# gtonkinhill/tracs

Hardware: NVIDIA B200
Metric: site-pair comparisons/s (P*L/t) (higher is better)
Workload: dtype u32 bit-planes (int32 counts), f64 likelihood

## Files before the change

### tracs_b200/csrc/sweep.cu

```cuda
#include <cub/cub.cuh>

#include <algorithm>
#include <memory>
#include <stdexcept>
#include <type_traits>

#include "common.cuh"
#include "trans.cuh"

namespace tracs {

static inline uint64_t round_up(uint64_t x, uint64_t m) { return (x + m - 1) / m * m; }

constexpr int PACK_THREADS = 256;
constexpr int PACK_SCHUNK = 256;
constexpr int PACK_BATCH = 4;

__device__ __forceinline__ uint32_t bsel(uint32_t a, uint32_t b, uint32_t m) { return (a & m) | (b & ~m); }

__device__ __forceinline__ uint32_t nibbles_all_ones(uint32_t x) {
  uint32_t t = x & (x >> 1);
  t &= (t >> 2);
  t &= 0x11111111u;
  t = (t | (t >> 3)) & 0x03030303u;
// ... 386 lines not shown
__global__ void k_site_sources(const uint32_t *__restrict__ vlist, uint32_t V, const uint32_t *__restrict__ elist, uint32_t VE,
                               uint32_t *__restrict__ src, uint32_t *__restrict__ late) {
  const uint32_t v = blockIdx.x * blockDim.x + threadIdx.x;
  if (v >= V) return;
  const uint32_t site = vlist[v];
  uint32_t a = 0, b = VE;
  while (a < b) {
    const uint32_t mid = (a + b) >> 1;
    if (elist[mid] < site) a = mid + 1; else b = mid;
  }
  if (a < VE && elist[a] == site) {
    src[v] = a;
  } else {
    src[v] = 0x80000000u | (v - a);
    late[v - a] = site;
  }
}

__device__ __forceinline__ uint32_t slice_bits4(uint32_t r, int b) {
  return (((r >> b) & 0x01010101u) * 0x01020408u) >> 24;
}
__device__ __forceinline__ uint4 slice_word(const uint4 &q0, const uint4 &q1) {
  const uint32_t r[8] = {q0.x, q0.y, q0.z, q0.w, q1.x, q1.y, q1.z, q1.w};
  uint32_t o[4];
#pragma unroll
  for (int b = 0; b < 4; ++b) {
    uint32_t v = 0;
#pragma unroll
    for (int k = 0; k < 8; ++k) v |= (slice_bits4(r[k], b) & 0xFu) << (4 * k);
    o[b] = v;
  }
  return make_uint4(o[0], o[1], o[2], o[3]);
}
__device__ __forceinline__ bool slice_ambiguous(const uint4 &p) {
  const uint32_t two = (p.x & p.y) | (p.x & p.z) | (p.x & p.w) | (p.y & p.z) | (p.y & p.w) | (p.z & p.w);
  return (two & ~(p.x & p.y & p.z & p.w)) != 0u;
}

__global__ void __launch_bounds__(256)
k_slice(const uint8_t *__restrict__ X, uint64_t XP, const uint8_t *__restrict__ X2, uint64_t X2P, const uint32_t *__restrict__ src,
        uint64_t V, uint64_t n, uint4 *__restrict__ planes, uint64_t Npad, uint4 *__restrict__ planesT, uint64_t Wp, uint32_t schunk,
        uint32_t *__restrict__ amb_flag) {
  const uint32_t lane = threadIdx.x & 31;
  const uint64_t w0 = ((uint64_t)blockIdx.x * 8 + (threadIdx.x >> 5)) * 2;
  if (w0 * 32 >= V) return;
  const uint64_t s0 = (uint64_t)blockIdx.y * schunk, s1 = min(n, s0 + schunk);
  bool fast = (w0 + 2) * 32 <= V;
  uint32_t base = 0;
  if (fast) {
    const uint32_t a = src[w0 * 32 + lane], b = src[w0 * 32 + 32 + lane];
    base = __shfl_sync(0xFFFFFFFFu, a, 0);
    fast = __all_sync(0xFFFFFFFFu, a == base + lane && b == base + 32 + lane) && !(base & 0x80000000u) && (base & 15u) == 0;
  }
  if (fast) {
    bool amb = false, hasn = false;
    for (uint64_t s = s0 + lane; s < s1; s += 32) {
      const uint4 *row = reinterpret_cast<const uint4 *>(X + s * XP + base);
      const uint4 q0 = __ldg(row), q1 = __ldg(row + 1), q2 = __ldg(row + 2), q3 = __ldg(row + 3);
      const uint4 pa = slice_word(q0, q1), pb = slice_word(q2, q3);
      amb |= slice_ambiguous(pa) | slice_ambiguous(pb);
      hasn |= ((pa.x & pa.y & pa.z & pa.w) | (pb.x & pb.y & pb.z & pb.w)) != 0u;
      planes[w0 * Npad + s] = pa;
      planes[(w0 + 1) * Npad + s] = pb;
      planesT[s * Wp + w0] = pa;
      planesT[s * Wp + w0 + 1] = pb;
    }
    if (__any_sync(0xFFFFFFFFu, amb) && lane == 0) atomicOr(amb_flag, 1u);
    if (__any_sync(0xFFFFFFFFu, hasn) && lane == 0) atomicOr(amb_flag, 2u);
    return;
  }
  for (uint64_t w = w0; w < w0 + 2 && w * 32 < V; ++w) {
    const uint64_t v = w * 32 + lane;
    const bool live = v < V;
    const uint32_t sv = live ? src[v] : 0u;
    const uint8_t *col = (sv & 0x80000000u) ? X2 + (sv & 0x7FFFFFFFu) : X + sv;
    const uint64_t cp = (sv & 0x80000000u) ? X2P : XP;
    constexpr int GB = 8;
    for (uint64_t sb = s0; sb < s1; sb += GB) {
      uint8_t mk[GB];
#pragma unroll
      for (int t = 0; t < GB; ++t) mk[t] = (live && sb + t < s1) ? __ldg(col + (sb + t) * cp) : (uint8_t)15;
#pragma unroll
      for (int t = 0; t < GB; ++t) {
        const uint64_t s = sb + t;
        if (s >= s1) break;
        const uint32_t m = mk[t];
        if (__any_sync(0xFFFFFFFFu, m != 15u && (m & (m - 1)) != 0u) && lane == 0) atomicOr(amb_flag, 1u);
        if (__any_sync(0xFFFFFFFFu, live && m == 15u) && lane == 0) atomicOr(amb_flag, 2u);
        const uint32_t A = __ballot_sync(0xFFFFFFFFu, m & 1);
        const uint32_t C = __ballot_sync(0xFFFFFFFFu, m & 2);
        const uint32_t G = __ballot_sync(0xFFFFFFFFu, m & 4);
        const uint32_t T = __ballot_sync(0xFFFFFFFFu, m & 8);
        if (lane == 0) {
          const uint4 o = make_uint4(A, C, G, T);
          planes[w * Npad + s] = o;
          planesT[s * Wp + w] = o;
        }
      }
    }
  }
}

struct SweepArgs {
  const uint4 *planes;
  uint32_t Wp;
  uint32_t Npad;
  uint32_t n, i_end, j_start;
  int32_t dist;
  const uint32_t *rb_list;
  const uint32_t *tile_prefix;
  uint32_t n_rb;
  uint32_t n_tiles;
  uint32_t cb_min;
  const uint2 *tile_table;
  const uint32_t *tc_ncnt;
  union {
    struct {
      unsigned long long *counter;
      uint64_t *keys;
      uint32_t *dvals;
      unsigned long long cap;
    };
    struct {
      int32_t *dense;
      uint64_t dense_ld;
      uint32_t dense_col0;
      uint32_t dense_mirror;
    };
  };
  uint32_t one;
};

__device__ __forceinline__ uint32_t smem_u32(const void *p) { return (uint32_t)__cvta_generic_to_shared(p); }
__device__ __forceinline__ void mbar_init(uint64_t *bar, uint32_t count) {
  asm volatile("mbarrier.init.shared::cta.b64 [%0], %1;" ::"r"(smem_u32(bar)), "r"(count) : "memory");
}
__device__ __forceinline__ void mbar_expect_tx(uint64_t *bar, uint32_t bytes) {
  asm volatile("mbarrier.arrive.expect_tx.shared::cta.b64 _, [%0], %1;" ::"r"(smem_u32(bar)), "r"(bytes) : "memory");
}
__device__ __forceinline__ void mbar_wait(uint64_t *bar, uint32_t parity) {
  uint32_t done;
  do {
    asm volatile(
        "{\n"
        ".reg .pred p;\n"
        "mbarrier.try_wait.parity.shared::cta.b64 p, [%1], %2;\n"
        "selp.u32 %0, 1, 0, p;\n"
        "}\n"
        : "=r"(done)
        : "r"(smem_u32(bar)), "r"(parity)
        : "memory");
  } while (!done);
}
__device__ __forceinline__ void bulk_g2s(void *dst, const void *src, uint32_t bytes, uint64_t *bar) {
  asm volatile("cp.async.bulk.shared::cluster.global.mbarrier::complete_tx::bytes [%0], [%1], %2, [%3];" ::"r"(
                   smem_u32(dst)),
               "l"(src), "r"(bytes), "r"(smem_u32(bar))
               : "memory");
}

__global__ void k_tile_table(const uint32_t *__restrict__ rb_list, const uint32_t *__restrict__ tile_prefix, uint32_t n_rb, uint32_t cb_min,
                             uint32_t n_tiles, uint2 *__restrict__ table) {
  const uint32_t tile = blockIdx.x * blockDim.x + threadIdx.x;
  if (tile >= n_tiles) return;
  uint32_t lo = 0, hi = n_rb;
  while (hi - lo > 1) {
    const uint32_t mid = (lo + hi) >> 1;
    if (tile_prefix[mid] <= tile) lo = mid; else hi = mid;
  }
  const uint32_t rb = rb_list[lo];
  table[tile] = make_uint2(rb, max(rb, cb_min) + (tile - tile_prefix[lo]));
}

constexpr int SWEEP_THREADS = 256;
constexpr int STAGE_U4 = KC * TILE;
constexpr uint32_t PREFILTER_WORDS = 64;
static inline uint32_t prefilter_words(int64_t dist) {
  const uint64_t w = ((uint64_t)(dist + 1) * 8 + 31) / 32;
  return (uint32_t)std::min<uint64_t>(PREFILTER_WORDS, std::max<uint64_t>(16, round_up(w, 16)));
}
static inline uint32_t first_window(int64_t dist) {
  if (dist < 22) return 4;
  if (dist < 43) return 8;
  return prefilter_words(dist);
}
constexpr uint32_t TC_MIN_WORDS = 17;
static inline uint32_t next_window(uint32_t pw) { return pw < 8 ? 8 : pw < 16 ? 16 : (pw < PREFILTER_WORDS ? PREFILTER_WORDS : 0); }
constexpr size_t SWEEP_SMEM = (size_t)STAGES * 2 * STAGE_U4 * sizeof(uint4);

extern __shared__ __align__(128) uint8_t smem_raw[];

template <bool DENSE>
__global__ void __launch_bounds__(SWEEP_THREADS, 1) k_sweep(const SweepArgs a) {
  extern __shared__ __align__(128) uint8_t smem_raw[];
  uint4 *srow = reinterpret_cast<uint4 *>(smem_raw);
  uint4 *scol = srow + (size_t)STAGES * STAGE_U4;
  __shared__ __align__(8) uint64_t full[STAGES];
  __shared__ uint2 s_tile[4];
  constexpr uint32_t HB_CAP = 1024, HB_FLUSH = 512, HB_LANE_MAX = 4;
  __shared__ uint64_t hb_key[HB_CAP];
  __shared__ uint32_t hb_val[HB_CAP];
  __shared__ uint32_t hb_count;
  __shared__ unsigned long long hb_base;

  const uint32_t tid = threadIdx.x;
  const uint32_t tx = tid & 15, ty = tid >> 4;
  if (tid == 0) {
    for (int s = 0; s < STAGES; ++s) mbar_init(&full[s], 1);
    asm volatile("fence.mbarrier_init.release.cluster;" ::: "memory");
    hb_count = 0;
  }
  __syncthreads();
  auto flush_hits = [&]() {
    const uint32_t cnt = hb_count;
    if (tid == 0) hb_base = cnt ? atomicAdd(a.counter, (unsigned long long)cnt) : 0ull;
    __syncthreads();
    const unsigned long long base = hb_base;
    for (uint32_t e = tid; e < cnt; e += SWEEP_THREADS)
      if (base + e < a.cap) {
        a.keys[base + e] = hb_key[e];
        a.dvals[base + e] = hb_val[e];
      }
    __syncthreads();
    if (tid == 0) hb_count = 0;
    __syncthreads();
  };

  const uint32_t nk = (a.Wp + KC - 1) / KC;
  const int kc_used = a.Wp < (uint32_t)KC ? (int)a.Wp : KC;
  const uint32_t one = a.one;
  const uint32_t my_tiles = blockIdx.x < a.n_tiles ? (a.n_tiles - blockIdx.x + gridDim.x - 1) / gridDim.x : 0;
  const uint32_t total_chunks = my_tiles * nk;
  const uint32_t warp_id = tid >> 5, lane_id = tid & 31;
  uint32_t iss_g = 0, iss_t = 0, iss_c = 0, iss_slot = 0;
  uint2 rc_next = my_tiles ? __ldg(a.tile_table + blockIdx.x) : make_uint2(0u, 0u);
  auto issue = [&]() {
    const uint2 rc = rc_next;
    uint64_t *bar = &full[iss_slot];
    if (lane_id == 0) {
      if (iss_c == 0) s_tile[iss_t & 3] = rc;
      mbar_expect_tx(bar, 2u * STAGE_U4 * (uint32_t)sizeof(uint4));
    }
    __syncwarp();
    if (lane_id < 2u * KC) {
      const uint32_t kk = lane_id >> 1;
      const bool is_col = (lane_id & 1u) != 0u;
      const uint4 *src = a.planes + (size_t)(is_col ? rc.y : rc.x) * TILE + (size_t)(iss_c * KC + kk) * a.Npad;
      uint4 *dst = (is_col ? scol : srow) + (size_t)iss_slot * STAGE_U4 + kk * TILE;
      bulk_g2s(dst, src, TILE * sizeof(uint4), bar);
    }
    ++iss_g;
    iss_slot = iss_slot + 1 == (uint32_t)STAGES ? 0u : iss_slot + 1;
    if (++iss_c == nk) {
      iss_c = 0;
      if (++iss_t < my_tiles) rc_next = __ldg(a.tile_table + blockIdx.x + (size_t)iss_t * gridDim.x);
    }
  };
  if (warp_id == 0)
    while (iss_g < (uint32_t)STAGES && iss_g < total_chunks) issue();
  __syncthreads();
  uint32_t it = 0;
  uint32_t t_iter = 0;

  for (uint32_t tile = blockIdx.x; tile < a.n_tiles; tile += gridDim.x, ++t_iter) {
    const uint2 rc = s_tile[t_iter & 3];
    const uint32_t rb = rc.x, cb = rc.y;

    uint32_t acc[8][8];
#pragma unroll
    for (int i = 0; i < 8; ++i)
#pragma unroll
      for (int j = 0; j < 8; ++j) acc[i][j] = 0;

    for (uint32_t c = 0; c < nk; ++c, ++it) {
      const uint32_t slot = it % STAGES;
      mbar_wait(&full[slot], (it / STAGES) & 1u);
      const uint4 *pr = srow + (size_t)slot * STAGE_U4 + ty;
      const uint4 *pc = scol + (size_t)slot * STAGE_U4 + tx;
#pragma unroll 2
      for (int kk = 0; kk < kc_used; ++kk) {
        uint4 r[8];
#pragma unroll
        for (int i = 0; i < 8; ++i) r[i] = pr[kk * TILE + i * 16];
#pragma unroll
        for (int j = 0; j < 8; ++j) {
          const uint4 cv = pc[kk * TILE + j * 16];
#pragma unroll
          for (int i = 0; i < 8; ++i) {
            const uint32_t m = (r[i].x & cv.x) | (r[i].y & cv.y) | (r[i].z & cv.z) | (r[i].w & cv.w);
            acc[i][j] = __popc(m) * one + acc[i][j];
          }
        }
      }
      const int want_flush = c + 1 == nk && *(volatile uint32_t *)&hb_count > HB_FLUSH;
      const int do_flush = __syncthreads_or(want_flush);
      if (warp_id == 0 && iss_g < total_chunks) issue();
      if (do_flush) flush_hits();
    }

    const uint32_t total_bits = a.Wp * 32u;
    if constexpr (DENSE) {
#pragma unroll
      for (int i = 0; i < 8; ++i) {
        const uint32_t gi = rb * TILE + i * 16 + ty;
#pragma unroll
        for (int j = 0; j < 8; ++j) {
          const uint32_t gj = cb * TILE + j * 16 + tx;
          if (gi < a.i_end && gj < a.n && gj > gi && gj >= a.j_start) {
            const int32_t d = (int32_t)(total_bits - acc[i][j]);
            a.dense[(uint64_t)gi * a.dense_ld + (gj - a.dense_col0)] = d;
            if (a.dense_mirror) a.dense[(uint64_t)gj * a.dense_ld + gi] = d;
          }
        }
        if (a.dense_mirror && cb == rb && tx == ty && gi < a.n) a.dense[(uint64_t)gi * a.dense_ld + gi] = 0;
      }
      continue;
    }
    const uint32_t lane = tid & 31;
    uint32_t rmax[8];
#pragma unroll
    for (int i = 0; i < 8; ++i) {
      uint32_t m = acc[i][0];
#pragma unroll
      for (int j = 1; j < 8; ++j) m = max(m, acc[i][j]);
      rmax[i] = m;
    }
    uint32_t mx = rmax[0];
#pragma unroll
    for (int i = 1; i < 8; ++i) mx = max(mx, rmax[i]);
    const bool hit = (int32_t)(total_bits - mx) <= a.dist;
    const uint32_t hits = __ballot_sync(0xFFFFFFFFu, hit);
    if (!hits) continue;
    if (__popc(hits) <= 8) {
      if (hit) {
        uint32_t rowmask = 0;
#pragma unroll
        for (int i = 0; i < 8; ++i) rowmask |= ((int32_t)(total_bits - rmax[i]) <= a.dist ? 1u : 0u) << i;
        uint32_t parked = 0;
        while (rowmask) {
          const int i = __ffs(rowmask) - 1;
          rowmask &= rowmask - 1;
          uint32_t rv[8];
#pragma unroll
          for (int j = 0; j < 8; ++j) {
            uint32_t v = acc[0][j];
#pragma unroll
            for (int ii = 1; ii < 8; ++ii) v = i == ii ? acc[ii][j] : v;
            rv[j] = v;
          }
          const uint32_t gi = rb * TILE + (uint32_t)i * 16 + ty;
          uint32_t keepj = 0;
#pragma unroll
          for (int j = 0; j < 8; ++j) {
            const uint32_t gj = cb * TILE + j * 16 + tx;
            const bool ok = (int32_t)(total_bits - rv[j]) <= a.dist && gi < a.i_end && gj < a.n && gj > gi && gj >= a.j_start;
            keepj |= (ok ? 1u : 0u) << j;
          }
          while (keepj) {
            const int j = __ffs(keepj) - 1;
            keepj &= keepj - 1;
            uint32_t v = rv[0];
#pragma unroll
            for (int jj = 1; jj < 8; ++jj) v = j == jj ? rv[jj] : v;
            const uint64_t key = ((uint64_t)gi << 32) | (cb * TILE + (uint32_t)j * 16 + tx);
            if (parked < HB_LANE_MAX) {
              const uint32_t pos = atomicAdd(&hb_count, 1u);
              hb_key[pos] = key;
              hb_val[pos] = total_bits - v;
              ++parked;
            } else {
              const unsigned long long pos = atomicAdd(a.counter, 1ull);
              if (pos < a.cap) {
                a.keys[pos] = key;
                a.dvals[pos] = total_bits - v;
              }
            }
          }
        }
      }
      continue;
    }
    uint32_t cnt = 0;
    uint64_t keep = 0;
#pragma unroll
    for (int i = 0; i < 8; ++i) {
      const uint32_t gi = rb * TILE + i * 16 + ty;
#pragma unroll
      for (int j = 0; j < 8; ++j) {
        const uint32_t gj = cb * TILE + j * 16 + tx;
        const int32_t d = (int32_t)(total_bits - acc[i][j]);
        const bool ok = gi < a.i_end && gj < a.n && gj > gi && gj >= a.j_start && d <= a.dist;
        if (ok) {
          keep |= 1ull << (i * 8 + j);
          cnt++;
        }
      }
    }
    uint32_t incl = cnt;
#pragma unroll
    for (int o = 1; o < 32; o <<= 1) {
      uint32_t t = __shfl_up_sync(0xFFFFFFFFu, incl, o);
      if (lane >= (uint32_t)o) incl += t;
    }
    const uint32_t wtot = __shfl_sync(0xFFFFFFFFu, incl, 31);
    if (wtot) {
      unsigned long long base = 0;
      if (lane == 31) base = atomicAdd(a.counter, (unsigned long long)wtot);
      base = __shfl_sync(0xFFFFFFFFu, base, 31);
      unsigned long long pos = base + (incl - cnt);
#pragma unroll
      for (int i = 0; i < 8; ++i) {
#pragma unroll
        for (int j = 0; j < 8; ++j) {
          if ((keep >> (i * 8 + j)) & 1ull) {
            if (pos < a.cap) {
              const uint32_t gi = rb * TILE + i * 16 + ty;
              const uint32_t gj = cb * TILE + j * 16 + tx;
              a.keys[pos] = ((uint64_t)gi << 32) | gj;
              a.dvals[pos] = total_bits - acc[i][j];
            }
            pos++;
          }
        }
      }
    }
  }
  __syncthreads();
  flush_hits();
}

__global__ void k_expand(const uint64_t *__restrict__ keys, const uint32_t *__restrict__ dvals, uint64_t E,
                         uint64_t *__restrict__ rows, uint64_t *__restrict__ cols, uint64_t *__restrict__ dist) {
  uint64_t e = (uint64_t)blockIdx.x * blockDim.x + threadIdx.x;
  if (e >= E) return;
  uint64_t k = keys[e];
  rows[e] = k >> 32;
  cols[e] = k & 0xFFFFFFFFull;
  dist[e] = dvals[e];
}

__global__ void __launch_bounds__(256)
k_refine(const uint64_t *__restrict__ ckeys, const uint32_t *__restrict__ cdvals, uint64_t n_cand,
         const uint4 *__restrict__ planesT, uint32_t Wp, uint32_t w0, int32_t dist, unsigned long long *counter,
         uint64_t *__restrict__ keys, uint32_t *__restrict__ dvals) {
  const uint64_t e = ((uint64_t)blockIdx.x * blockDim.x + threadIdx.x) >> 5;
  const uint32_t lane = threadIdx.x & 31;
  if (e >= n_cand) return;
  const uint64_t k = ckeys[e];
  const uint4 *ri = planesT + (k >> 32) * Wp;
  const uint4 *rj = planesT + (k & 0xFFFFFFFFull) * Wp;
  uint32_t mism = 0;
#pragma unroll 4
  for (uint32_t w = w0 + lane; w < Wp; w += 32) {
    const uint4 x = __ldg(ri + w), y = __ldg(rj + w);
    mism += __popc(~((x.x & y.x) | (x.y & y.y) | (x.z & y.z) | (x.w & y.w)));
  }
#pragma unroll
  for (int o = 16; o > 0; o >>= 1) mism += __shfl_xor_sync(0xFFFFFFFFu, mism, o);
  if (lane == 0) {
    const uint32_t d = cdvals[e] + mism;
    if ((int32_t)d <= dist) {
      const unsigned long long pos = atomicAdd(counter, 1ull);
      keys[pos] = k;
      dvals[pos] = d;
    }
  }
}

__global__ void __launch_bounds__(256)
k_cand_trim(const uint64_t *__restrict__ keys, const uint32_t *__restrict__ dvals, uint64_t n_cand, const uint4 *__restrict__ planesT,
            uint32_t Wp, uint32_t w0, uint32_t extra, int32_t dist, uint8_t *__restrict__ flags) {
  const uint64_t e = (uint64_t)blockIdx.x * blockDim.x + threadIdx.x;
  if (e >= n_cand) return;
  const uint64_t k = keys[e];
  const uint4 *ri = planesT + (k >> 32) * Wp + w0, *rj = planesT + (k & 0xFFFFFFFFull) * Wp + w0;
  uint32_t d = dvals[e];
  for (uint32_t w = 0; w < extra && (int32_t)d <= dist; w += 4) {
#pragma unroll
    for (uint32_t q = 0; q < 4; ++q) {
      if (w + q < extra) {
        const uint4 x = __ldg(ri + w + q), y = __ldg(rj + w + q);
        d += __popc(~((x.x & y.x) | (x.y & y.y) | (x.z & y.z) | (x.w & y.w)));
      }
    }
  }
  flags[e] = (int32_t)d <= dist ? 1 : 0;
}

__global__ void __launch_bounds__(256)
k_snp_positions(const uint64_t *__restrict__ keys, uint64_t e0, uint64_t e1, const uint4 *__restrict__ planesT, uint32_t Wp,
                const uint32_t *__restrict__ site_idx, uint64_t V, const uint64_t *__restrict__ offs, uint64_t base,
                uint32_t *__restrict__ pos) {
  const uint64_t e = e0 + (((uint64_t)blockIdx.x * blockDim.x + threadIdx.x) >> 5);
  const uint32_t lane = threadIdx.x & 31;
  if (e >= e1) return;
  const uint64_t k = keys[e];
  const uint4 *ri = planesT + (k >> 32) * Wp;
  const uint4 *rj = planesT + (k & 0xFFFFFFFFull) * Wp;
  uint32_t *out = pos + (offs[e] - base);
  uint32_t written = 0;
  for (uint32_t w0 = 0; w0 < Wp; w0 += 32) {
    const uint32_t w = w0 + lane;
    uint32_t mis = 0;
    if (w < Wp) {
      const uint4 x = __ldg(ri + w), y = __ldg(rj + w);
      mis = ~((x.x & y.x) | (x.y & y.y) | (x.z & y.z) | (x.w & y.w));
    }
    const uint32_t c = __popc(mis);
    uint32_t incl = c;
#pragma unroll
    for (int o = 1; o < 32; o <<= 1) {
      const uint32_t t = __shfl_up_sync(0xFFFFFFFFu, incl, o);
      if (lane >= (uint32_t)o) incl += t;
    }
    uint32_t at = written + incl - c;
    while (mis) {
      const uint32_t b = __ffs(mis) - 1;
      mis &= mis - 1;
      const uint64_t v = (uint64_t)w * 32 + b;
      out[at++] = v < V ? site_idx[v] : 0u;
    }
    written += __shfl_sync(0xFFFFFFFFu, incl, 31);
  }
}

__global__ void __launch_bounds__(256)
k_filter_recomb(const uint32_t *__restrict__ dvals, uint64_t e0, uint64_t e1, const uint64_t *__restrict__ offs, uint64_t base,
                const uint32_t *__restrict__ pos, uint64_t L, const double *__restrict__ lg, uint32_t *__restrict__ filt) {
  const uint64_t e = e0 + (((uint64_t)blockIdx.x * blockDim.x + threadIdx.x) >> 5);
  const uint32_t lane = threadIdx.x & 31;
  if (e >= e1) return;
  const uint32_t d = dvals[e];
  if (d <= 1) {
    if (lane == 0) filt[e] = d;
    return;
  }
  const uint32_t *ps = pos + (offs[e] - base);
  const int aln = (int)L;
  const double dd = (double)d;
  const double p = dd / aln, thr = 0.05 / dd;
  int h = (int)(1.0 / p / 2.0 + 1);
  h = min(h, 5000);
  h = max(h, 50);
  const double lp = log(p), lq = log1p(-p);
  uint32_t kept = 0;
  for (uint32_t s = lane; s < d; s += 32) {
    const int i = (int)ps[s];
    const int left = max(0, i - h), right = min(aln, i + h + 1);
    uint32_t lo = 0, hi = s;
    while (lo < hi) { const uint32_t m = (lo + hi) >> 1; if ((int)ps[m] < left) lo = m + 1; else hi = m; }
    const uint32_t a = lo;
    lo = s; hi = d;
    while (lo < hi) { const uint32_t m = (lo + hi) >> 1; if ((int)ps[m] < right) lo = m + 1; else hi = m; }
    const uint32_t b = lo;
    const uint32_t cnt = b - a;
    if (cnt > 1) {
      const double n = (double)(int)(ps[b - 1] - ps[a] + 1), kk = (double)(int)cnt;
      double cdf;
      if (kk >= n) cdf = 1.0;
      else {
        cdf = 0.0;
        const int ni = (int)n;
        for (int t = 0; t <= (int)cnt; ++t)
          cdf += exp(lg[ni + 1] - lg[t + 1] - lg[ni - t + 1] + (double)t * lp + (double)(ni - t) * lq);
        if (cdf > 1.0) cdf = 1.0;
      }
      if (1.0 - cdf >= thr) kept++;
    } else {
      kept++;
    }
  }
#pragma unroll
  for (int o = 16; o > 0; o >>= 1) kept += __shfl_xor_sync(0xFFFFFFFFu, kept, o);
  if (lane == 0) filt[e] = kept;
}
__global__ void k_pack_edges(const uint64_t *__restrict__ keys, const uint32_t *__restrict__ dvals, const uint64_t *__restrict__ ncomp,
                             const double *__restrict__ p0, const double *__restrict__ eK, uint64_t E, uint8_t *__restrict__ out) {
  const uint64_t e = (uint64_t)blockIdx.x * blockDim.x + threadIdx.x;
  if (e >= E) return;
  uint32_t *u = reinterpret_cast<uint32_t *>(out);
  double *f = reinterpret_cast<double *>(out + 16 * E);
  const uint64_t k = keys[e];
  u[e] = (uint32_t)(k >> 32);
  u[E + e] = (uint32_t)k;
  u[2 * E + e] = dvals[e];
  u[3 * E + e] = ncomp ? (uint32_t)ncomp[e] : 0u;
  f[e] = p0 ? p0[e] : 0.0;
  f[E + e] = eK ? eK[e] : 0.0;
}
struct WidenU32 {
  __host__ __device__ __forceinline__ uint64_t operator()(const uint32_t &v) const { return (uint64_t)v; }
};
__global__ void k_widen(const uint32_t *__restrict__ in, uint64_t E, uint64_t *__restrict__ out) {
  const uint64_t e = (uint64_t)blockIdx.x * blockDim.x + threadIdx.x;
  if (e < E) out[e] = in[e];
}

__global__ void k_rep_init(uint32_t *rep, uint32_t n) {
  uint32_t s = blockIdx.x * blockDim.x + threadIdx.x;
  if (s < n) rep[s] = s;
}
__global__ void k_rep_min(const uint64_t *__restrict__ keys, uint64_t E, uint32_t *rep) {
  const uint64_t e = (uint64_t)blockIdx.x * blockDim.x + threadIdx.x;
  if (e >= E) return;
  const uint64_t k = keys[e];
  atomicMin(rep + (k & 0xFFFFFFFFull), (uint32_t)(k >> 32));
}
__global__ void k_rep_keys(const uint64_t *__restrict__ keys, uint64_t E, const uint32_t *__restrict__ rep,
                           uint32_t *__restrict__ okey, uint32_t *__restrict__ oval) {
  const uint64_t e = (uint64_t)blockIdx.x * blockDim.x + threadIdx.x;
  if (e >= E) return;
  okey[e] = rep[keys[e] >> 32];
  oval[e] = (uint32_t)e;
}

__global__ void __launch_bounds__(256)
k_ncomp(const uint64_t *__restrict__ keys, uint64_t E, const uint32_t *__restrict__ nplane, uint64_t npitch,
        const uint8_t *__restrict__ nsum, uint64_t spitch, const uint32_t *__restrict__ ncount, uint64_t L,
        const uint32_t *__restrict__ order, uint64_t *__restrict__ ncomp) {
  const uint64_t slot = ((uint64_t)blockIdx.x * blockDim.x + threadIdx.x) >> 5;
  const uint32_t lane = threadIdx.x & 31;
  if (slot >= E) return;
  const uint64_t e = order ? order[slot] : slot;
  const uint64_t k = keys[e];
  const uint64_t i = k >> 32, j = k & 0xFFFFFFFFull;
  const uint32_t *si = reinterpret_cast<const uint32_t *>(nsum + i * spitch);
  const uint32_t *sj = reinterpret_cast<const uint32_t *>(nsum + j * spitch);
  const uint4 *ni = reinterpret_cast<const uint4 *>(nplane + i * npitch);
  const uint4 *nj = reinterpret_cast<const uint4 *>(nplane + j * npitch);
  uint32_t inter = 0;
  const uint64_t nq = spitch / 4;
  for (uint64_t q = lane; q < nq; q += 32) {
    uint32_t m = __ldg(si + q) & __ldg(sj + q);
    while (m) {
      uint32_t b = __ffs(m) - 1;
      m &= m - 1;
      uint64_t blk = q * 32 + b;
      uint4 x = __ldg(ni + blk), y = __ldg(nj + blk);
      inter += __popc(x.x & y.x) + __popc(x.y & y.y) + __popc(x.z & y.z) + __popc(x.w & y.w);
    }
  }
#pragma unroll
  for (int o = 16; o > 0; o >>= 1) inter += __shfl_xor_sync(0xFFFFFFFFu, inter, o);
  if (lane == 0) ncomp[e] = L - ((uint64_t)ncount[i] + ncount[j] - inter);
}

__global__ void k_trans_mark(const uint64_t *__restrict__ keys, const uint32_t *__restrict__ dvals, uint64_t E,
                             const uint64_t *__restrict__ E_dev, const int32_t *__restrict__ days, uint32_t DD,
                             uint8_t *__restrict__ used) {
  const uint64_t e = (uint64_t)blockIdx.x * blockDim.x + threadIdx.x;
  if (e >= (E_dev ? *E_dev : E)) return;
  const uint64_t k = keys[e];
  const int32_t dd = abs(days[k >> 32] - days[k & 0xFFFFFFFFull]);
  uint8_t *u = used + (uint64_t)dvals[e] * DD + (uint32_t)dd;
  if (!*u) *u = 1;
}
__global__ void k_trans_table(const uint32_t *__restrict__ key_idx, const uint64_t *__restrict__ n_keys, uint64_t n_all, uint32_t DD,
                              const double *__restrict__ lg, double lamb, double beta, double thr,
                              double *__restrict__ p0_lut, double *__restrict__ eK_lut) {
  const uint64_t t = (uint64_t)blockIdx.x * blockDim.x + threadIdx.x;
  if (t >= (key_idx ? *n_keys : n_all)) return;
  const uint32_t id = key_idx ? key_idx[t] : (uint32_t)t;
  const double delta = ((double)(id % DD) * 86400.0) / 31556952.0;
  trans_eval((int64_t)(id / DD), delta, lg, lamb, beta, thr, &p0_lut[id], &eK_lut[id]);
}
__global__ void k_trans_gather(const uint64_t *__restrict__ keys, const uint32_t *__restrict__ dvals, uint64_t E,
                               const uint64_t *__restrict__ E_dev, const int32_t *__restrict__ days, uint32_t DD,
                               const double *__restrict__ p0_lut, const double *__restrict__ eK_lut, double *__restrict__ p0,
                               double *__restrict__ eK, double *__restrict__ dt) {
  const uint64_t e = (uint64_t)blockIdx.x * blockDim.x + threadIdx.x;
  if (e >= (E_dev ? *E_dev : E)) return;
  const uint64_t k = keys[e];
  const int32_t dd = abs(days[k >> 32] - days[k & 0xFFFFFFFFull]);
  const uint64_t id = (uint64_t)dvals[e] * DD + (uint32_t)dd;
  p0[e] = p0_lut[id];
  eK[e] = eK_lut[id];
  dt[e] = ((double)dd * 86400.0) / 31556952.0;
}

}
#include "sweep_tc3.inl"
namespace tracs {

static void launch_tile_sweep(const SweepArgs &a_in, bool use_tc, cudaStream_t st, bool has_n, bool dense) {
  SweepArgs a = a_in;
  TRACS_CK(cudaFuncSetAttribute(k_sweep<false>, cudaFuncAttributeMaxDynamicSharedMemorySize, (int)SWEEP_SMEM));
  TRACS_CK(cudaFuncSetAttribute(k_sweep<true>, cudaFuncAttributeMaxDynamicSharedMemorySize, (int)SWEEP_SMEM));
  int dev = 0, n_sm = 148;
  cudaGetDevice(&dev);
  cudaDeviceGetAttribute(&n_sm, cudaDevAttrMultiProcessorCount, dev);
  if (a.n_tiles == 0) return;
  g_stats.tc_sweep = use_tc ? 30.0f + (has_n ? 4.0f : 3.0f) : 0.0f;
  if (use_tc) {
    DevBuf<uint32_t> ncnt;
    a.tc_ncnt = nullptr;
    if (has_n) {
      ncnt.alloc(a.Npad);
      k_tc_ncount<<<(a.Npad + 255) / 256, 256, 0, st>>>(a.planes, a.Npad, a.Wp, ncnt.p);
      g_stats.kernel_launches++;
      a.tc_ncnt = ncnt.p;
    }
    TRACS_CK(cudaFuncSetAttribute(k_sweep_tc3<3>, cudaFuncAttributeMaxDynamicSharedMemorySize, (int)Tc3Geom<3>::SMEM));
    TRACS_CK(cudaFuncSetAttribute(k_sweep_tc3<4>, cudaFuncAttributeMaxDynamicSharedMemorySize, (int)Tc3Geom<4>::SMEM));
    TRACS_CK(cudaFuncSetAttribute((k_sweep_tc3<3, true>), cudaFuncAttributeMaxDynamicSharedMemorySize, (int)Tc3Geom<3>::SMEM));
    TRACS_CK(cudaFuncSetAttribute((k_sweep_tc3<4, true>), cudaFuncAttributeMaxDynamicSharedMemorySize, (int)Tc3Geom<4>::SMEM));
    std::vector<uint32_t> h_prefix(a.n_rb + 1), sprefix(a.n_rb + 1, 0);
    TRACS_CK(cudaMemcpyAsync(h_prefix.data(), a.tile_prefix, (a.n_rb + 1) * 4, cudaMemcpyDeviceToHost, st));
    TRACS_CK(cudaStreamSynchronize(st));
    for (uint32_t k = 0; k < a.n_rb; ++k) sprefix[k + 1] = sprefix[k] + (h_prefix[k + 1] - h_prefix[k] + 3) / 4;
    const uint32_t n_stiles = sprefix[a.n_rb];
    DevBuf<uint32_t> d_sprefix(a.n_rb + 1);
    DevBuf<uint2> d_stiles(std::max<uint32_t>(1, n_stiles));
    TRACS_CK(cudaMemcpyAsync(d_sprefix.p, sprefix.data(), (a.n_rb + 1) * 4, cudaMemcpyHostToDevice, st));
    k_stile_table<<<(n_stiles + 255) / 256, 256, 0, st>>>(a.rb_list, d_sprefix.p, a.n_rb, a.cb_min, a.Npad / TILE, n_stiles, d_stiles.p);
    g_stats.kernel_launches++;
    const unsigned grid = (unsigned)std::min<uint64_t>(n_stiles, (uint64_t)n_sm);
    const char *dbg_env = getenv("TRACS_TC3_DBG");
    const uint32_t dbg = dbg_env ? (uint32_t)atoi(dbg_env) : 0u;
    if (dense && has_n) k_sweep_tc3<4, true><<<grid, TC3_THREADS, Tc3Geom<4>::SMEM, st>>>(a, d_stiles.p, n_stiles, dbg);
    else if (dense) k_sweep_tc3<3, true><<<grid, TC3_THREADS, Tc3Geom<3>::SMEM, st>>>(a, d_stiles.p, n_stiles, dbg);
    else if (has_n) k_sweep_tc3<4><<<grid, TC3_THREADS, Tc3Geom<4>::SMEM, st>>>(a, d_stiles.p, n_stiles, dbg);
    else k_sweep_tc3<3><<<grid, TC3_THREADS, Tc3Geom<3>::SMEM, st>>>(a, d_stiles.p, n_stiles, dbg);
    TRACS_CK(cudaStreamSynchronize(st));
  } else {
    int occ = 1;
    cudaOccupancyMaxActiveBlocksPerMultiprocessor(&occ, k_sweep<false>, SWEEP_THREADS, SWEEP_SMEM);
    const unsigned grid = (unsigned)std::min<uint64_t>(a.n_tiles, (uint64_t)n_sm * std::max(1, occ));
    if (dense) k_sweep<true><<<grid, SWEEP_THREADS, SWEEP_SMEM, st>>>(a);
    else k_sweep<false><<<grid, SWEEP_THREADS, SWEEP_SMEM, st>>>(a);
  }
  g_stats.kernel_launches++;
  TRACS_CK(cudaGetLastError());
}



struct Ingested {
  uint64_t n = 0, L = 0;
  uint64_t npitch = 0, spitch = 0;
  uint64_t V = 0, W = 0;
  uint32_t Wp = KC, Npad = 0;
  DevBuf<uint32_t> nplane, ncount, site_idx;
  DevBuf<uint8_t> nsum;
  DevBuf<uint4> planes, planesT;
  bool partial_ambiguity = false;
  uint64_t n_total = 0;
  bool has_n_var = true;
  bool nplane_sparse = false;
};

__global__ void k_sum_u32(const uint32_t *__restrict__ v, uint64_t n, unsigned long long *out) {
  unsigned long long s = 0;
  for (uint64_t i = (uint64_t)blockIdx.x * blockDim.x + threadIdx.x; i < n; i += (uint64_t)gridDim.x * blockDim.x) s += v[i];
#pragma unroll
  for (int o = 16; o > 0; o >>= 1) s += __shfl_xor_sync(0xFFFFFFFFu, s, o);
  if ((threadIdx.x & 31) == 0 && s) atomicAdd(out, s);
}

static void ingest_device(const uint8_t *dev_seqs, uint64_t n, uint64_t L, uint64_t pitch, bool packed, bool keep_site_idx,
                          Ingested &g, cudaStream_t st, uint64_t rows_before = 0, DevBuf<uint32_t> *keep_colmask = nullptr) {
  tracs_stats_t &S = g_stats;
  if (!packed && (pitch % 32 != 0 || pitch < round_up(L, 32)))
    throw std::runtime_error("device alignment pitch must be a multiple of 32 and >= L rounded up to 32");
  if (packed && (pitch % 16 != 0 || pitch * 2 < std::max<uint64_t>(32, round_up(L, 32))))
    throw std::runtime_error("packed alignment pitch must be a multiple of 16 bytes and hold L rounded up to 32 sites");
  Timer T(st);
  g.n = n;
  g.L = L;
  const uint64_t Lw = (L + 31) / 32;
  const uint64_t npitch = std::max<uint64_t>(32, round_up(Lw, 32));
  const uint64_t spitch = round_up(npitch / 32, 4);
  g.npitch = npitch;
  g.spitch = spitch;
  DevBuf<uint32_t> colmask(std::max<uint64_t>(1, Lw * 4));
  DevBuf<uint32_t> &nplane = g.nplane, &ncount = g.ncount;
  DevBuf<uint8_t> &nsum = g.nsum;
  const char *mode_env = getenv("TRACS_INGEST");
  const uint64_t n_first = PACK_SCHUNK;
  bool early = L >= (1u << 16) && n >= 4 * n_first && L < (1ull << 31);
  if (mode_env && !strcmp(mode_env, "split")) early = false;
  if (mode_env && !strcmp(mode_env, "early")) early = L > 0 && n > n_first && L < (1ull << 31);
  const char *np_env = getenv("TRACS_NPLANE");
  const char *nb_env = getenv("TRACS_NBLOCKS");
  const bool sparse_candidate = early && !(np_env && !strcmp(np_env, "always")) && !(nb_env && !strcmp(nb_env, "dense"));
  g.nplane_sparse = false;
  nplane.alloc((rows_before + n) * npitch);
  nsum.alloc((rows_before + n) * spitch);
  ncount.alloc(rows_before + n);
  uint32_t *const np0 = nplane.p + rows_before * npitch, *const nc0 = ncount.p + rows_before;
  uint8_t *const ns0 = nsum.p + rows_before * spitch;
  const uint32_t Npad = (uint32_t)round_up(n, TILE);
  DevBuf<uint32_t> &site_idx = g.site_idx;
  T.start();
  TRACS_CK(cudaMemsetAsync(colmask.p, 0xFF, colmask.n * sizeof(uint32_t), st));
  TRACS_CK(cudaMemsetAsync(nsum.p, 0, nsum.n, st));
  TRACS_CK(cudaMemsetAsync(ncount.p, 0, ncount.n * sizeof(uint32_t), st));

  auto select_sites = [&](DevBuf<uint32_t> &list) -> uint64_t {
    DevBuf<uint8_t> flags(round_up(L, 8));
    k_siteflags<<<(unsigned)((Lw * 4 + 255) / 256), 256, 0, st>>>(colmask.p, L, flags.p);
    list.alloc(L);
    DevBuf<uint64_t> nsel(1);
    size_t tmp_bytes = 0;
    cub::CountingInputIterator<uint32_t> cnt_it(0);
    cub::DeviceSelect::Flagged(nullptr, tmp_bytes, cnt_it, flags.p, list.p, nsel.p, (int64_t)L, st);
    DevBuf<uint8_t> tmp(tmp_bytes);
    cub::DeviceSelect::Flagged(tmp.p, tmp_bytes, cnt_it, flags.p, list.p, nsel.p, (int64_t)L, st);
    S.kernel_launches += 3;
    uint64_t cnt = 0;
    TRACS_CK(cudaMemcpyAsync(&cnt, nsel.p, sizeof(uint64_t), cudaMemcpyDeviceToHost, st));
    TRACS_CK(cudaStreamSynchronize(st));
    return cnt;
  };
  auto launch_pack = [&](uint64_t sa, uint64_t sb, const uint32_t *elist, uint32_t VE, uint8_t *X, uint64_t XP) {
    if (sb <= sa) return;
    dim3 grid((unsigned)((npitch + PACK_THREADS - 1) / PACK_THREADS), (unsigned)((sb - sa + PACK_SCHUNK - 1) / PACK_SCHUNK));
    if (packed) {
      if (VE && g.nplane_sparse) {
        TRACS_CK(cudaFuncSetAttribute((k_pack4<true, true>), cudaFuncAttributePreferredSharedMemoryCarveout, 60));
        k_pack4<true, true><<<grid, PACK_THREADS, 0, st>>>(dev_seqs, sa, sb, L, pitch, colmask.p, np0, npitch, ns0, spitch,
                                                         nc0, elist, VE, X, XP);
      } else if (VE) {
        TRACS_CK(cudaFuncSetAttribute((k_pack4<true, false>), cudaFuncAttributePreferredSharedMemoryCarveout, 60));
        k_pack4<true><<<grid, PACK_THREADS, 0, st>>>(dev_seqs, sa, sb, L, pitch, colmask.p, np0, npitch, ns0, spitch, nc0,
                                                   elist, VE, X, XP);
      } else {
        k_pack4<false><<<grid, PACK_THREADS, 0, st>>>(dev_seqs, sa, sb, L, pitch, colmask.p, np0, npitch, ns0, spitch, nc0,
                                                    nullptr, 0, nullptr, 0);
      }
    } else if (VE) {
      TRACS_CK(cudaFuncSetAttribute(k_pack_x<false>, cudaFuncAttributePreferredSharedMemoryCarveout, 60));
      TRACS_CK(cudaFuncSetAttribute(k_pack_x<true>, cudaFuncAttributePreferredSharedMemoryCarveout, 60));
      if (g.nplane_sparse)
        k_pack_x<true><<<grid, PACK_THREADS, 0, st>>>(dev_seqs, sa, sb, L, pitch, colmask.p, np0, npitch, ns0, spitch, nc0,
                                                    elist, VE, X, XP);
      else
        k_pack_x<false><<<grid, PACK_THREADS, 0, st>>>(dev_seqs, sa, sb, L, pitch, colmask.p, np0, npitch, ns0, spitch, nc0,
                                                     elist, VE, X, XP);
    } else {
      k_pack<<<grid, PACK_THREADS, 0, st>>>(dev_seqs, sa, sb, L, pitch, colmask.p, np0, npitch, ns0, spitch, nc0);
    }
    S.kernel_launches++;
    TRACS_CK(cudaGetLastError());
  };
  DevBuf<uint32_t> elist;
  DevBuf<uint8_t> X;
  uint64_t VE = 0, XP = 0;
  if (L == 0) {
    TRACS_CK(cudaMemsetAsync(nplane.p, 0, nplane.n * sizeof(uint32_t), st));
  } else if (!early) {
    Timer Tm(st);
    Tm.start();
    launch_pack(0, n, nullptr, 0, nullptr, 0);
    S.ms_pack_main += Tm.stop();
  } else {
    launch_pack(0, n_first, nullptr, 0, nullptr, 0);
    std::vector<uint32_t> first_cnt(sparse_candidate ? n_first : 0);
    if (sparse_candidate)
      TRACS_CK(cudaMemcpyAsync(first_cnt.data(), nc0, n_first * sizeof(uint32_t), cudaMemcpyDeviceToHost, st));
    VE = select_sites(elist);
    if (VE > L / 16) VE = 0;
    if (VE) {
      XP = round_up(VE, 32);
      X.alloc(n * XP);
    } else {
      early = false;
    }
    if (sparse_candidate && VE) {
      double tot = 0;
      for (uint32_t c : first_cnt) tot += c;
      const double p_n = tot / ((double)n_first * (double)L);
      g.nplane_sparse = 1.0 - pow(1.0 - std::min(1.0, p_n), 128.0) <= 0.35;
      if (np_env && !strcmp(np_env, "sparse")) g.nplane_sparse = true;
      if (g.nplane_sparse) S.sparse_nplane = 1.0f;
    }
    Timer Tm(st);
// ... 623 lines not shown
```

Before: 273000000 billion.

## Add narrow-window sweep variant with per-warp empty barriers and warp-local hit queues

Adds a NARROW specialization of the popcount sweep for thresholded runs where the packed width equals four words. It uses an 8-slot TMA ring in which each warp owns refills for one slot, gated by per-slot empty mbarriers, replacing the block-wide __syncthreads_or per chunk. Hit buffering moves to per-warp queues flushed with warp-level atomics, so no block barrier is needed for output either. The aim is to remove block-wide synchronization that dominates when each tile has only one short k-chunk. The cost is more intricate barrier parity logic and deferred refill issue, which risks stalls if a warp falls behind.

```diff
diff --git a/tracs_b200/csrc/sweep.cu b/tracs_b200/csrc/sweep.cu
--- a/tracs_b200/csrc/sweep.cu
+++ b/tracs_b200/csrc/sweep.cu
@@ -562,6 +562,22 @@
         : "memory");
   } while (!done);
 }
+__device__ __forceinline__ void mbar_arrive(uint64_t *bar) {
+  asm volatile("mbarrier.arrive.shared::cta.b64 _, [%0];" ::"r"(smem_u32(bar)) : "memory");
+}
+__device__ __forceinline__ bool mbar_test(uint64_t *bar, uint32_t parity) {
+  uint32_t done;
+  asm volatile(
+      "{\n"
+      ".reg .pred p;\n"
+      "mbarrier.test_wait.parity.shared::cta.b64 p, [%1], %2;\n"
+      "selp.u32 %0, 1, 0, p;\n"
+      "}\n"
+      : "=r"(done)
+      : "r"(smem_u32(bar)), "r"(parity)
+      : "memory");
+  return done != 0u;
+}
 __device__ __forceinline__ void bulk_g2s(void *dst, const void *src, uint32_t bytes, uint64_t *bar) {
   asm volatile("cp.async.bulk.shared::cluster.global.mbarrier::complete_tx::bytes [%0], [%1], %2, [%3];" ::"r"(
                    smem_u32(dst)),
@@ -597,17 +613,29 @@
 constexpr uint32_t TC_MIN_WORDS = 17;
 static inline uint32_t next_window(uint32_t pw) { return pw < 8 ? 8 : pw < 16 ? 16 : (pw < PREFILTER_WORDS ? PREFILTER_WORDS : 0); }
 constexpr size_t SWEEP_SMEM = (size_t)STAGES * 2 * STAGE_U4 * sizeof(uint4);
+constexpr int NARROW_KC = 4;
+constexpr int NARROW_STAGES = 8;
+constexpr int NARROW_STAGE_U4 = NARROW_KC * TILE;
+constexpr size_t NARROW_SMEM = (size_t)NARROW_STAGES * 2 * NARROW_STAGE_U4 * sizeof(uint4);
+static_assert(NARROW_STAGES == SWEEP_THREADS / 32, "every warp owns the refills of one ring slot");
 
 extern __shared__ __align__(128) uint8_t smem_raw[];
 
-template <bool DENSE>
+template <bool DENSE, bool NARROW = false>
 __global__ void __launch_bounds__(SWEEP_THREADS, 1) k_sweep(const SweepArgs a) {
+  static_assert(!(DENSE && NARROW), "the narrow ring serves thresholded sweeps only");
+  constexpr int NS = NARROW ? NARROW_STAGES : STAGES;
+  constexpr int SU4 = NARROW ? NARROW_STAGE_U4 : STAGE_U4;
   extern __shared__ __align__(128) uint8_t smem_raw[];
   uint4 *srow = reinterpret_cast<uint4 *>(smem_raw);
-  uint4 *scol = srow + (size_t)STAGES * STAGE_U4;
-  __shared__ __align__(8) uint64_t full[STAGES];
+  uint4 *scol = srow + (size_t)NS * SU4;
+  __shared__ __align__(8) uint64_t full[NS];
   __shared__ uint2 s_tile[4];
+  __shared__ __align__(8) uint64_t n_empty[NARROW_STAGES];
+  __shared__ uint2 n_tile[NARROW_STAGES];
+  __shared__ uint32_t wq_count[SWEEP_THREADS / 32];
   constexpr uint32_t HB_CAP = 1024, HB_FLUSH = 512, HB_LANE_MAX = 4;
+  constexpr uint32_t WQ_CAP = HB_CAP / (SWEEP_THREADS / 32), WQ_FLUSH = WQ_CAP - 8 * HB_LANE_MAX;
   __shared__ uint64_t hb_key[HB_CAP];
   __shared__ uint32_t hb_val[HB_CAP];
   __shared__ uint32_t hb_count;
@@ -616,10 +644,14 @@
   const uint32_t tid = threadIdx.x;
   const uint32_t tx = tid & 15, ty = tid >> 4;
   if (tid == 0) {
-    for (int s = 0; s < STAGES; ++s) mbar_init(&full[s], 1);
+    for (int s = 0; s < NS; ++s) mbar_init(&full[s], 1);
+    if constexpr (NARROW)
+      for (int s = 0; s < NS; ++s) mbar_init(&n_empty[s], SWEEP_THREADS / 32);
     asm volatile("fence.mbarrier_init.release.cluster;" ::: "memory");
     hb_count = 0;
   }
+  if constexpr (NARROW)
+    if (tid < SWEEP_THREADS / 32) wq_count[tid] = 0;
   __syncthreads();
   auto flush_hits = [&]() {
     const uint32_t cnt = hb_count;
@@ -635,8 +667,24 @@
     if (tid == 0) hb_count = 0;
     __syncthreads();
   };
-
-  const uint32_t nk = (a.Wp + KC - 1) / KC;
+  const uint32_t wq0 = NARROW ? (tid >> 5) * WQ_CAP : 0u;
+  auto flush_queue = [&]() {
+    __syncwarp();
+    const uint32_t cnt = wq_count[tid >> 5];
+    unsigned long long base = 0;
+    if ((tid & 31) == 0 && cnt) base = atomicAdd(a.counter, (unsigned long long)cnt);
+    base = __shfl_sync(0xFFFFFFFFu, base, 0);
+    for (uint32_t e = tid & 31; e < cnt; e += 32)
+      if (base + e < a.cap) {
+        a.keys[base + e] = hb_key[wq0 + e];
+        a.dvals[base + e] = hb_val[wq0 + e];
+      }
+    __syncwarp();
+    if ((tid & 31) == 0) wq_count[tid >> 5] = 0;
+    __syncwarp();
+  };
+
+  const uint32_t nk = NARROW ? 1u : (a.Wp + KC - 1) / KC;
   const int kc_used = a.Wp < (uint32_t)KC ? (int)a.Wp : KC;
   const uint32_t one = a.one;
   const uint32_t my_tiles = blockIdx.x < a.n_tiles ? (a.n_tiles - blockIdx.x + gridDim.x - 1) / gridDim.x : 0;
@@ -666,14 +714,54 @@
       if (++iss_t < my_tiles) rc_next = __ldg(a.tile_table + blockIdx.x + (size_t)iss_t * gridDim.x);
     }
   };
-  if (warp_id == 0)
-    while (iss_g < (uint32_t)STAGES && iss_g < total_chunks) issue();
+  auto issue_narrow = [&](uint32_t t, uint2 rc) {
+    const uint32_t slot = t % NS;
+    if (lane_id == 0) {
+      n_tile[slot] = rc;
+      mbar_expect_tx(&full[slot], 2u * SU4 * (uint32_t)sizeof(uint4));
+    }
+    __syncwarp();
+    if (lane_id < 2u * NARROW_KC) {
+      const uint32_t kk = lane_id >> 1;
+      const bool is_col = (lane_id & 1u) != 0u;
+      const uint4 *src = a.planes + (size_t)(is_col ? rc.y : rc.x) * TILE + (size_t)kk * a.Npad;
+      uint4 *dst = (is_col ? scol : srow) + (size_t)slot * SU4 + kk * TILE;
+      bulk_g2s(dst, src, TILE * sizeof(uint4), &full[slot]);
+    }
+  };
+  if constexpr (NARROW) {
+    if (warp_id == 0)
+      for (uint32_t t = 0; t < (uint32_t)NS && t < my_tiles; ++t) issue_narrow(t, __ldg(a.tile_table + blockIdx.x + (size_t)t * gridDim.x));
+  } else {
+    if (warp_id == 0)
+      while (iss_g < (uint32_t)STAGES && iss_g < total_chunks) issue();
+  }
   __syncthreads();
   uint32_t it = 0;
   uint32_t t_iter = 0;
+  uint32_t owed = ~0u;
+  uint2 rc_owed = make_uint2(0u, 0u);
 
   for (uint32_t tile = blockIdx.x; tile < a.n_tiles; tile += gridDim.x, ++t_iter) {
-    const uint2 rc = s_tile[t_iter & 3];
+    uint2 rc;
+    if constexpr (NARROW) {
+      if (owed != ~0u) {
+        const uint32_t par = (owed / NS - 1u) & 1u;
+        bool ready = __shfl_sync(0xFFFFFFFFu, mbar_test(&n_empty[warp_id], par), 0);
+        if (!ready && owed == t_iter) {
+          mbar_wait(&n_empty[warp_id], par);
+          ready = true;
+        }
+        if (ready) {
+          issue_narrow(owed, rc_owed);
+          owed = ~0u;
+        }
+      }
+      mbar_wait(&full[t_iter % NS], (t_iter / NS) & 1u);
+      rc = n_tile[t_iter % NS];
+    } else {
+      rc = s_tile[t_iter & 3];
+    }
     const uint32_t rb = rc.x, cb = rc.y;
 
     uint32_t acc[8][8];
@@ -683,10 +771,10 @@
       for (int j = 0; j < 8; ++j) acc[i][j] = 0;
 
     for (uint32_t c = 0; c < nk; ++c, ++it) {
-      const uint32_t slot = it % STAGES;
-      mbar_wait(&full[slot], (it / STAGES) & 1u);
-      const uint4 *pr = srow + (size_t)slot * STAGE_U4 + ty;
-      const uint4 *pc = scol + (size_t)slot * STAGE_U4 + tx;
+      const uint32_t slot = it % NS;
+      if constexpr (!NARROW) mbar_wait(&full[slot], (it / NS) & 1u);
+      const uint4 *pr = srow + (size_t)slot * SU4 + ty;
+      const uint4 *pc = scol + (size_t)slot * SU4 + tx;
 #pragma unroll 2
       for (int kk = 0; kk < kc_used; ++kk) {
         uint4 r[8];
@@ -702,10 +790,19 @@
           }
         }
       }
-      const int want_flush = c + 1 == nk && *(volatile uint32_t *)&hb_count > HB_FLUSH;
-      const int do_flush = __syncthreads_or(want_flush);
-      if (warp_id == 0 && iss_g < total_chunks) issue();
-      if (do_flush) flush_hits();
+      if constexpr (NARROW) {
+        __syncwarp();
+        if (lane_id == 0) mbar_arrive(&n_empty[slot]);
+        if (slot == warp_id && t_iter + NS < my_tiles) {
+          owed = t_iter + NS;
+          rc_owed = __ldg(a.tile_table + blockIdx.x + (size_t)owed * gridDim.x);
+        }
+      } else {
+        const int want_flush = c + 1 == nk && *(volatile uint32_t *)&hb_count > HB_FLUSH;
+        const int do_flush = __syncthreads_or(want_flush);
+        if (warp_id == 0 && iss_g < total_chunks) issue();
+        if (do_flush) flush_hits();
+      }
     }
 
     const uint32_t total_bits = a.Wp * 32u;
@@ -774,7 +871,7 @@
             for (int jj = 1; jj < 8; ++jj) v = j == jj ? rv[jj] : v;
             const uint64_t key = ((uint64_t)gi << 32) | (cb * TILE + (uint32_t)j * 16 + tx);
             if (parked < HB_LANE_MAX) {
-              const uint32_t pos = atomicAdd(&hb_count, 1u);
+              const uint32_t pos = NARROW ? wq0 + atomicAdd(&wq_count[warp_id], 1u) : atomicAdd(&hb_count, 1u);
               hb_key[pos] = key;
               hb_val[pos] = total_bits - v;
               ++parked;
@@ -788,6 +885,10 @@
           }
         }
       }
+      if constexpr (NARROW) {
+        __syncwarp();
+        if (wq_count[warp_id] > WQ_FLUSH) flush_queue();
+      }
       continue;
     }
     uint32_t cnt = 0;
@@ -835,8 +936,12 @@
       }
     }
   }
-  __syncthreads();
-  flush_hits();
+  if constexpr (NARROW) {
+    flush_queue();
+  } else {
+    __syncthreads();
+    flush_hits();
+  }
 }
 
 __global__ void k_expand(const uint64_t *__restrict__ keys, const uint32_t *__restrict__ dvals, uint64_t E,
@@ -1132,6 +1237,12 @@
     else if (has_n) k_sweep_tc3<4><<<grid, TC3_THREADS, Tc3Geom<4>::SMEM, st>>>(a, d_stiles.p, n_stiles, dbg);
     else k_sweep_tc3<3><<<grid, TC3_THREADS, Tc3Geom<3>::SMEM, st>>>(a, d_stiles.p, n_stiles, dbg);
     TRACS_CK(cudaStreamSynchronize(st));
+  } else if (!dense && a.Wp == (uint32_t)NARROW_KC) {
+    TRACS_CK(cudaFuncSetAttribute((k_sweep<false, true>), cudaFuncAttributeMaxDynamicSharedMemorySize, (int)NARROW_SMEM));
+    int occ = 1;
+    cudaOccupancyMaxActiveBlocksPerMultiprocessor(&occ, k_sweep<false, true>, SWEEP_THREADS, NARROW_SMEM);
+    const unsigned grid = (unsigned)std::min<uint64_t>(a.n_tiles, (uint64_t)n_sm * std::max(1, occ));
+    k_sweep<false, true><<<grid, SWEEP_THREADS, NARROW_SMEM, st>>>(a);
   } else {
     int occ = 1;
     cudaOccupancyMaxActiveBlocksPerMultiprocessor(&occ, k_sweep<false>, SWEEP_THREADS, SWEEP_SMEM);
```

Measured after the change: 277200000 billion (median of 6 runs). +1.5%, better.
